# fluidex/plonkit

Measured on AMD Instinct MI355X. Metric: G1 MSM throughput at 2^20 terms per GPU (KZG commitment of the PLONK prover), higher is better.
Workload: dtype u256 (BN254 Fr/Fq Montgomery; 9x29-bit limbs in registers, v_mad_u64_u32); 1 GPU; Pippenger G1 MSM (KZG commitment), 2^20 uniform scalars per GPU, tau=42 monomial SRS sharded by rank (BASELINE configs[1]); terms_per_gpu=1048576, parallelism=srs-shard x1 + all_gather of partial sums, exchange=none (one GPU), pipeline_depth=3, settle_steps=0, comm_ranks=1

## Files before the change

### plonkit_amd/csrc/ec29_dev.h

```cpp
#pragma once
#include "field29_dev.h"
#include "ec_dev.h"

namespace plk {

struct AffW { FqW9 x, y; };
struct alignas(16) XyzzW { FqW9 x, y, zz, zzz; };

#define WM(a, b) mulw<FqW>((a), (b))
#define WS(a) sqrw<FqW>((a))
#define WMA(a, b, c, d) mul2addw<FqW>((a), (b), (c), (d))
#define LM(a, b) mulw_os<FqW>((a), (b))
#define LS(a) sqrw_os<FqW>((a))
#define LMA(a, b, c, d) mul2addw_os<FqW>((a), (b), (c), (d))

PLK_HD bool is_inf(const XyzzW &p) { return w_all_zero(p.zz); }
PLK_HD bool is_inf(const AffW &p) { return w_all_zero(p.x) && w_all_zero(p.y); }
PLK_HD XyzzW xyzzw_identity() { XyzzW r; r.x = w_zero<FqW>(); r.y = w_zero<FqW>(); r.zz = w_zero<FqW>(); r.zzz = w_zero<FqW>(); return r; }

PLK_HD XyzzW xyzzw_double_affine(const FqW9 &x, const FqW9 &y) {
    FqW9 u = addn(y, y), v = WS(u), w = WM(u, v), s = WM(x, v);
    FqW9 xx = WS(x), m = normw(addw(addw(xx, xx), xx));
    XyzzW r;
    r.x = sub4(WS(m), addn(s, s));
    r.y = WMA(m, sub6(s, r.x), y, neg2(w));
    r.zz = v; r.zzz = w;
    return r;
}

PLK_HD XyzzW xyzzw_double(const XyzzW &p) {
    if (is_inf(p)) return p;
    FqW9 u = addn(p.y, p.y), v = LS(u), w = LM(u, v), s = LM(p.x, v);
    FqW9 xx = LS(p.x), m = normw(addw(addw(xx, xx), xx));
    XyzzW r;
    r.x = sub4(LS(m), addn(s, s));
    r.y = LMA(m, sub6(s, r.x), p.y, neg2(w));
    r.zz = LM(v, p.zz); r.zzz = LM(w, p.zzz);
    return r;
}

PLK_HD void xyzzw_add(XyzzW &a, const XyzzW &b);
PLK_HD void xyzzw_add_mixed_special(XyzzW &acc, const AffW &q, bool neg_q, const FqW9 &p, const FqW9 &r) {
    if (is_zero_mod_p(p)) {
        if (is_zero_mod_p(r)) acc = xyzzw_double_affine(q.x, neg_q ? neg2(q.y) : q.y);
        else acc = xyzzw_identity();
        return;
    }
    XyzzW t; t.x = q.x; t.y = neg_q ? neg2(q.y) : q.y; t.zz = w_one<FqW>(); t.zzz = w_one<FqW>();
    xyzzw_add(acc, t);
}

PLK_HD void xyzzw_add_mixed(XyzzW &acc, const AffW &q, bool neg_q) {
    if (is_inf(q)) return;
    if (is_inf(acc)) { acc.x = q.x; acc.y = neg_q ? neg2(q.y) : q.y; acc.zz = w_one<FqW>(); acc.zzz = w_one<FqW>(); return; }
    FqW9 u2, s2;
    mulw2<FqW>(q.x, acc.zz, q.y, acc.zzz, u2, s2);
    FqW9 p = sub6(u2, acc.x);
    FqW9 r;
    {
        const uint32_t m = neg_q ? 0xffffffffu : 0u;
#pragma unroll
        for (int i = 0; i < 9; i++) r.l[i] = FqW::PAD8[i] - acc.y.l[i] + ((s2.l[i] ^ m) - m);
        r = normw(r);
    }
    if (maybe_zero_mod_p(p)) {
        xyzzw_add_mixed_special(acc, q, neg_q, p, r);
        return;
    }
    FqW9 pp, rr, ppp, qq;
    sqrw2<FqW>(p, r, pp, rr);
    mulw2<FqW>(p, pp, acc.x, pp, ppp, qq);
    FqW9 x3;
    {
#pragma unroll
        for (int i = 0; i < 9; i++) x3.l[i] = rr.l[i] + FqW::PAD4[i] - ppp.l[i] - 2 * qq.l[i];
        x3 = normw(x3);
    }
    FqW9 zz3, zzz3;
    mulw2<FqW>(acc.zz, pp, acc.zzz, ppp, zz3, zzz3);
    acc.y = WMA(r, sub6(qq, x3), acc.y, neg2(ppp));
    acc.x = x3;
    acc.zz = zz3;
    acc.zzz = zzz3;
}

PLK_HD void xyzzw_add_mixed_flag(XyzzW &acc, bool &fresh, const AffW &q, bool neg_q) {
    if (fresh) { acc.x = q.x; acc.y = neg_q ? neg2(q.y) : q.y; acc.zz = w_one<FqW>(); acc.zzz = w_one<FqW>(); fresh = false; return; }
    FqW9 p, r, yq;
    {
        FqW9 ax, ay;
#pragma unroll
        for (int i = 0; i < 9; i++) {
            ax.l[i] = FqW::PAD6[i] - acc.x.l[i];
            ay.l[i] = FqW::PAD8[i] - acc.y.l[i];
            yq.l[i] = neg_q ? FqW::PAD2[i] - q.y.l[i] : q.y.l[i];
        }
        mulw2_add<FqW>(q.x, acc.zz, ax, yq, acc.zzz, ay, p, r);
    }
    if (maybe_zero_mod_p(p)) {
        AffW t; t.x = q.x; t.y = normw(yq);
        xyzzw_add_mixed_special(acc, t, false, p, r);
        fresh = is_inf(acc);
        return;
    }
    FqW9 pp, rr, ppp, qq;
    sqrw2<FqW>(p, r, pp, rr);
    mulw2<FqW>(p, pp, acc.x, pp, ppp, qq);
    FqW9 x3;
    {
#pragma unroll
        for (int i = 0; i < 9; i++) x3.l[i] = rr.l[i] + FqW::PAD4[i] - ppp.l[i] - 2 * qq.l[i];
        x3 = normw(x3);
    }
    FqW9 zz3, zzz3;
    mulw2<FqW>(acc.zz, pp, acc.zzz, ppp, zz3, zzz3);
    FqW9 t, nppp;
#pragma unroll
    for (int i = 0; i < 9; i++) { t.l[i] = qq.l[i] + FqW::PAD6N[i] - x3.l[i]; nppp.l[i] = FqW::PAD2N[i] - ppp.l[i]; }
    acc.y = WMA(r, t, acc.y, nppp);
    acc.x = x3;
    acc.zz = zz3;
    acc.zzz = zzz3;
}

PLK_HD void xyzzw_add(XyzzW &a, const XyzzW &b) {
    if (is_inf(b)) return;
    if (is_inf(a)) { a = b; return; }
    FqW9 u1 = LM(a.x, b.zz), u2 = LM(b.x, a.zz), s1 = LM(a.y, b.zzz), s2 = LM(b.y, a.zzz);
    FqW9 p = sub2(u2, u1), r = sub2(s2, s1);
    if (is_zero_mod_p(p)) {
        if (is_zero_mod_p(r)) a = xyzzw_double(a);
        else a = xyzzw_identity();
        return;
    }
    FqW9 pp = LS(p), ppp = LM(p, pp), qq = LM(u1, pp);
    FqW9 x3;
    {
        FqW9 rr = LS(r);
#pragma unroll
        for (int i = 0; i < 9; i++) x3.l[i] = rr.l[i] + FqW::PAD4[i] - ppp.l[i] - 2 * qq.l[i];
        x3 = normw(x3);
    }
    a.y = LMA(r, sub6(qq, x3), s1, neg2(ppp));
    a.x = x3;
    a.zz = LM(LM(a.zz, b.zz), pp);
    a.zzz = LM(LM(a.zzz, b.zzz), ppp);
}

PLK_HD void xyzzw_add_pairs(XyzzW &a, const XyzzW &b) {
    if (is_inf(b)) return;
    if (is_inf(a)) { a = b; return; }
    FqW9 u1, s1, p, r;
    mulw2<FqW>(a.x, b.zz, a.y, b.zzz, u1, s1);
    {
        FqW9 nu, ns;
#pragma unroll
        for (int i = 0; i < 9; i++) { nu.l[i] = FqW::PAD2[i] - u1.l[i]; ns.l[i] = FqW::PAD2[i] - s1.l[i]; }
        mulw2_add<FqW>(b.x, a.zz, nu, b.y, a.zzz, ns, p, r);
    }
    if (is_zero_mod_p(p)) {
        if (is_zero_mod_p(r)) a = xyzzw_double(a);
        else a = xyzzw_identity();
        return;
    }
    FqW9 zz12, zzz12;
    mulw2<FqW>(a.zz, b.zz, a.zzz, b.zzz, zz12, zzz12);
    FqW9 pp, rr, ppp, qq;
#pragma unroll
    for (int i = 0; i < 9; i++) { PLK_CHAIN(p.l[i]); PLK_CHAIN(r.l[i]); }
    sqrw2<FqW>(p, r, pp, rr);
    mulw2<FqW>(p, pp, u1, pp, ppp, qq);
    FqW9 x3;
    {
#pragma unroll
        for (int i = 0; i < 9; i++) x3.l[i] = rr.l[i] + FqW::PAD4[i] - ppp.l[i] - 2 * qq.l[i];
        x3 = normw(x3);
    }
    FqW9 t, nppp;
#pragma unroll
    for (int i = 0; i < 9; i++) { t.l[i] = qq.l[i] + FqW::PAD6N[i] - x3.l[i]; nppp.l[i] = FqW::PAD2N[i] - ppp.l[i]; }
    a.y = WMA(r, t, s1, nppp);
    a.x = x3;
    mulw2<FqW>(zz12, pp, zzz12, ppp, a.zz, a.zzz);
}

__device__ __forceinline__ AffW load_affw(const G1Affine *p) {
    AffW r; r.x = unpack<FqW>(load_fp(&p->x)); r.y = unpack<FqW>(load_fp(&p->y)); return r;
}
__device__ __forceinline__ FqW9 load_w(const uint32_t *p) {
    FqW9 r;
    const u32x4 *q = reinterpret_cast<const u32x4 *>(p);
    u32x4 a = q[0], b = q[1];
    r.l[0] = a.x; r.l[1] = a.y; r.l[2] = a.z; r.l[3] = a.w; r.l[4] = b.x; r.l[5] = b.y; r.l[6] = b.z; r.l[7] = b.w; r.l[8] = p[8];
    return r;
}
__device__ __forceinline__ void store_w(uint32_t *p, const FqW9 &v) {
    u32x4 *q = reinterpret_cast<u32x4 *>(p);
    q[0] = u32x4{v.l[0], v.l[1], v.l[2], v.l[3]};
    q[1] = u32x4{v.l[4], v.l[5], v.l[6], v.l[7]};
    p[8] = v.l[8];
}
__device__ __forceinline__ XyzzW load_xyzzw(const XyzzW *p) {
    const uint32_t *w = reinterpret_cast<const uint32_t *>(p);
    XyzzW r;
    FqW9 *c[4] = {&r.x, &r.y, &r.zz, &r.zzz};
    u32x4 tail = *reinterpret_cast<const u32x4 *>(w + 32);
    const uint32_t t[4] = {tail.x, tail.y, tail.z, tail.w};
#pragma unroll
    for (int k = 0; k < 4; k++) {
        const u32x4 *q = reinterpret_cast<const u32x4 *>(w + 8 * k);
        u32x4 a = q[0], b = q[1];
        c[k]->l[0] = a.x; c[k]->l[1] = a.y; c[k]->l[2] = a.z; c[k]->l[3] = a.w;
        c[k]->l[4] = b.x; c[k]->l[5] = b.y; c[k]->l[6] = b.z; c[k]->l[7] = b.w; c[k]->l[8] = t[k];
    }
    return r;
}
__device__ __forceinline__ void store_xyzzw(XyzzW *p, const XyzzW &v) {
    uint32_t *w = reinterpret_cast<uint32_t *>(p);
    const FqW9 *c[4] = {&v.x, &v.y, &v.zz, &v.zzz};
#pragma unroll
    for (int k = 0; k < 4; k++) {
        u32x4 *q = reinterpret_cast<u32x4 *>(w + 8 * k);
        q[0] = u32x4{c[k]->l[0], c[k]->l[1], c[k]->l[2], c[k]->l[3]};
        q[1] = u32x4{c[k]->l[4], c[k]->l[5], c[k]->l[6], c[k]->l[7]};
    }
    *reinterpret_cast<u32x4 *>(w + 32) = u32x4{v.x.l[8], v.y.l[8], v.zz.l[8], v.zzz.l[8]};
}

__device__ __forceinline__ G1Xyzz xyzzw_export(const XyzzW &p) {
    G1Xyzz r;
    if (is_inf(p)) return xyzz_identity();
    r.x = pack<FqParams>(s_from_w(p.x)); r.y = pack<FqParams>(s_from_w(p.y));
    r.zz = pack<FqParams>(s_from_w(p.zz)); r.zzz = pack<FqParams>(s_from_w(p.zzz));
    return r;
}

}
```

### plonkit_amd/csrc/field29_dev.h

```cpp
#pragma once
#include "field_dev.h"
#include <utility>

namespace plk {

template <int... J, class F> __device__ __forceinline__ void static_for_impl(std::integer_sequence<int, J...>, F &&f) { (f(std::integral_constant<int, J>{}), ...); }
template <int N, class F> __device__ __forceinline__ void static_for(F &&f) { static_for_impl(std::make_integer_sequence<int, N>{}, static_cast<F &&>(f)); }

constexpr uint32_t M29 = (1u << 29) - 1;
constexpr uint32_t MULW_A_LIMB_MAX = 3280000000u;

struct FrW {
    static constexpr uint32_t P29[9] = {0x10000001u, 0x1f0fac9fu, 0x0e5c2450u, 0x07d090f3u, 0x1585d283u, 0x02db40c0u, 0x00a6e141u, 0x0e5c2634u, 0x0030644eu};
    static constexpr uint32_t INV29 = 0x0fffffffu;
    static constexpr uint32_t PINV0 = 0x10000001u;
    static constexpr uint32_t ONE_W[9] = {0x0fffff57u, 0x1ea70ab4u, 0x052c068bu, 0x17504f49u, 0x0aa8075bu, 0x1d4240ceu, 0x11d54c07u, 0x052ac7a8u, 0x000dc836u};
    static constexpr uint32_t W_FROM_S[9] = {0x0fffead7u, 0x1d5444f4u, 0x04438aa5u, 0x03b4d096u, 0x134c84dau, 0x0e92d304u, 0x14cb95b3u, 0x041b9d3du, 0x00058003u};
    static constexpr uint32_t S_FROM_W[9] = {0x0ffffffbu, 0x04b1a0e2u, 0x18334a6bu, 0x18ed2b3eu, 0x1462e36fu, 0x11b7bc3cu, 0x1cbd99bau, 0x183340fbu, 0x000e0a77u};
    static constexpr uint32_t PAD2[9] = {0x80000002u, 0x9e1f593bu, 0x9cb8489du, 0x8fa121e2u, 0x8b0ba502u, 0x85b6817du, 0x814dc27eu, 0x9cb84c64u, 0x0060c898u};
    static constexpr uint32_t PAD4[9] = {0x80000004u, 0x9c3eb27au, 0x9970913fu, 0x9f4243c9u, 0x96174a08u, 0x8b6d02feu, 0x829b8500u, 0x997098ccu, 0x00c19135u};
    static constexpr uint32_t PAD6[9] = {0x80000006u, 0x9a5e0bb9u, 0x9628d9e1u, 0x8ee365b0u, 0x8122ef0fu, 0x91238480u, 0x83e94782u, 0x9628e534u, 0x012259d2u};
    static constexpr uint32_t PAD8[9] = {0x80000008u, 0x987d64f8u, 0x92e12283u, 0x9e848797u, 0x8c2e9415u, 0x96da0601u, 0x85370a04u, 0x92e1319cu, 0x0183226fu};
};

// ... 95 lines not shown
#pragma unroll
    for (int i = 0; i < 9; i++) r.l[i] = WP::PAD2[i] - a.l[i];
    return normw(r);
}
template <class WP> PLK_HD W9<WP> addn(const W9<WP> &a, const W9<WP> &b) { return normw(addw(a, b)); }

#if defined(__HIP_DEVICE_COMPILE__)
#define PLK_CHAIN(acc) asm("" : "+v"(acc))
#else
#define PLK_CHAIN(acc) do { } while (0)
#endif
#define PLK_MONT_LOW(k)  { _Pragma("unroll") for (int i = 0; i < (k); i++) { acc += (uint64_t)m[i] * WP::P29[(k) - i]; PLK_CHAIN(acc); } \
                           m[k] = ((uint32_t)acc * WP::INV29) & M29; acc += (uint64_t)m[k] * WP::P29[0]; acc >>= 29; }
#define PLK_MONT_HIGH(k) { _Pragma("unroll") for (int i = (k) - 8; i <= 8; i++) { acc += (uint64_t)m[i] * WP::P29[(k) - i]; PLK_CHAIN(acc); } \
                           r.l[(k) - 9] = (uint32_t)acc & M29; acc >>= 29; }
template <class WP>
PLK_HD W9<WP> mulw(const W9<WP> &a, const W9<WP> &b) {
    uint32_t m[9];
    W9<WP> r;
    uint64_t acc = 0;
#pragma unroll
    for (int k = 0; k < 9; k++) {
#pragma unroll
        for (int i = 0; i <= k; i++) { acc += (uint64_t)a.l[k - i] * b.l[i]; PLK_CHAIN(acc); }
        PLK_MONT_LOW(k)
    }
#pragma unroll
    for (int k = 9; k < 17; k++) {
#pragma unroll
        for (int i = k - 8; i <= 8; i++) { acc += (uint64_t)a.l[k - i] * b.l[i]; PLK_CHAIN(acc); }
        PLK_MONT_HIGH(k)
    }
    r.l[8] = (uint32_t)acc;
    return r;
}
#define PLK_MONT_LOW2(k)  { _Pragma("unroll") for (int i = 0; i < (k); i++) { acc0 += (uint64_t)m0[i] * WP::P29[(k) - i]; PLK_CHAIN(acc0); acc1 += (uint64_t)m1[i] * WP::P29[(k) - i]; PLK_CHAIN(acc1); } \
                            m0[k] = ((uint32_t)acc0 * WP::INV29) & M29; m1[k] = ((uint32_t)acc1 * WP::INV29) & M29; \
                            acc0 += (uint64_t)m0[k] * WP::P29[0]; acc1 += (uint64_t)m1[k] * WP::P29[0]; acc0 >>= 29; acc1 >>= 29; }
#define PLK_MONT_HIGH2(k) { _Pragma("unroll") for (int i = (k) - 8; i <= 8; i++) { acc0 += (uint64_t)m0[i] * WP::P29[(k) - i]; PLK_CHAIN(acc0); acc1 += (uint64_t)m1[i] * WP::P29[(k) - i]; PLK_CHAIN(acc1); } \
                            r0.l[(k) - 9] = (uint32_t)acc0 & M29; r1.l[(k) - 9] = (uint32_t)acc1 & M29; acc0 >>= 29; acc1 >>= 29; }
template <class WP>
PLK_HD void mulw2(const W9<WP> &a0, const W9<WP> &b0, const W9<WP> &a1, const W9<WP> &b1, W9<WP> &r0, W9<WP> &r1) {
    uint32_t m0[9], m1[9];
    uint64_t acc0 = 0, acc1 = 0;
#pragma unroll
    for (int k = 0; k < 9; k++) {
#pragma unroll
        for (int i = 0; i <= k; i++) { acc0 += (uint64_t)a0.l[k - i] * b0.l[i]; PLK_CHAIN(acc0); acc1 += (uint64_t)a1.l[k - i] * b1.l[i]; PLK_CHAIN(acc1); }
        PLK_MONT_LOW2(k)
    }
#pragma unroll
    for (int k = 9; k < 17; k++) {
#pragma unroll
        for (int i = k - 8; i <= 8; i++) { acc0 += (uint64_t)a0.l[k - i] * b0.l[i]; PLK_CHAIN(acc0); acc1 += (uint64_t)a1.l[k - i] * b1.l[i]; PLK_CHAIN(acc1); }
        PLK_MONT_HIGH2(k)
    }
    r0.l[8] = (uint32_t)acc0; r1.l[8] = (uint32_t)acc1;
}
template <class WP>
PLK_HD void sqrw2(const W9<WP> &x0, const W9<WP> &x1, W9<WP> &r0, W9<WP> &r1) {
    uint32_t m0[9], m1[9], d0[9], d1[9];
    uint64_t acc0 = 0, acc1 = 0;
#pragma unroll
    for (int j = 0; j < 9; j++) { d0[j] = x0.l[j] << 1; d1[j] = x1.l[j] << 1; }
#pragma unroll
    for (int k = 0; k < 9; k++) {
#pragma unroll
        for (int i = 0; 2 * i < k; i++) { acc0 += (uint64_t)d0[k - i] * x0.l[i]; PLK_CHAIN(acc0); acc1 += (uint64_t)d1[k - i] * x1.l[i]; PLK_CHAIN(acc1); }
        if (k % 2 == 0) { acc0 += (uint64_t)x0.l[k / 2] * x0.l[k / 2]; PLK_CHAIN(acc0); acc1 += (uint64_t)x1.l[k / 2] * x1.l[k / 2]; PLK_CHAIN(acc1); }
        PLK_MONT_LOW2(k)
    }
#pragma unroll
    for (int k = 9; k < 17; k++) {
#pragma unroll
        for (int i = k - 8; 2 * i < k; i++) { acc0 += (uint64_t)d0[k - i] * x0.l[i]; PLK_CHAIN(acc0); acc1 += (uint64_t)d1[k - i] * x1.l[i]; PLK_CHAIN(acc1); }
        if (k % 2 == 0) { acc0 += (uint64_t)x0.l[k / 2] * x0.l[k / 2]; PLK_CHAIN(acc0); acc1 += (uint64_t)x1.l[k / 2] * x1.l[k / 2]; PLK_CHAIN(acc1); }
        PLK_MONT_HIGH2(k)
    }
    r0.l[8] = (uint32_t)acc0; r1.l[8] = (uint32_t)acc1;
}
#if defined(__HIP_DEVICE_COMPILE__)
#define PLK_ADDEND(acc, x) { uint32_t one_ = 1; asm("" : "+s"(one_)); (acc) += (uint64_t)(x) * one_; }
#else
#define PLK_ADDEND(acc, x) { (acc) += (uint64_t)(x); }
#endif
#define PLK_MONT_HIGH2_ADD(k) { _Pragma("unroll") for (int i = (k) - 8; i <= 8; i++) { acc0 += (uint64_t)m0[i] * WP::P29[(k) - i]; PLK_CHAIN(acc0); acc1 += (uint64_t)m1[i] * WP::P29[(k) - i]; PLK_CHAIN(acc1); } \
                                PLK_ADDEND(acc0, A0.l[(k) - 9]); PLK_ADDEND(acc1, A1.l[(k) - 9]); \
                                r0.l[(k) - 9] = (uint32_t)acc0 & M29; r1.l[(k) - 9] = (uint32_t)acc1 & M29; acc0 >>= 29; acc1 >>= 29; }
template <class WP>
PLK_HD void mulw2_add(const W9<WP> &a0, const W9<WP> &b0, const W9<WP> &A0, const W9<WP> &a1, const W9<WP> &b1, const W9<WP> &A1, W9<WP> &r0, W9<WP> &r1) {
    uint32_t m0[9], m1[9];
    uint64_t acc0 = 0, acc1 = 0;
#pragma unroll
    for (int k = 0; k < 9; k++) {
#pragma unroll
        for (int i = 0; i <= k; i++) { acc0 += (uint64_t)a0.l[k - i] * b0.l[i]; PLK_CHAIN(acc0); acc1 += (uint64_t)a1.l[k - i] * b1.l[i]; PLK_CHAIN(acc1); }
        PLK_MONT_LOW2(k)
    }
#pragma unroll
    for (int k = 9; k < 17; k++) {
#pragma unroll
        for (int i = k - 8; i <= 8; i++) { acc0 += (uint64_t)a0.l[k - i] * b0.l[i]; PLK_CHAIN(acc0); acc1 += (uint64_t)a1.l[k - i] * b1.l[i]; PLK_CHAIN(acc1); }
        PLK_MONT_HIGH2_ADD(k)
    }
    r0.l[8] = (uint32_t)acc0 + A0.l[8]; r1.l[8] = (uint32_t)acc1 + A1.l[8];
}

template <class WP>
PLK_HD W9<WP> sqrw(const W9<WP> &a) {
    uint32_t m[9], a2[9];
    W9<WP> r;
    uint64_t acc = 0;
#pragma unroll
    for (int j = 0; j < 9; j++) a2[j] = a.l[j] << 1;
#pragma unroll
    for (int k = 0; k < 9; k++) {
#pragma unroll
        for (int i = 0; 2 * i < k; i++) { acc += (uint64_t)a2[k - i] * a.l[i]; PLK_CHAIN(acc); }
        if (k % 2 == 0) { acc += (uint64_t)a.l[k / 2] * a.l[k / 2]; PLK_CHAIN(acc); }
        PLK_MONT_LOW(k)
    }
#pragma unroll
    for (int k = 9; k < 17; k++) {
#pragma unroll
        for (int i = k - 8; 2 * i < k; i++) { acc += (uint64_t)a2[k - i] * a.l[i]; PLK_CHAIN(acc); }
        if (k % 2 == 0) { acc += (uint64_t)a.l[k / 2] * a.l[k / 2]; PLK_CHAIN(acc); }
        PLK_MONT_HIGH(k)
    }
    r.l[8] = (uint32_t)acc;
    return r;
}

template <class WP>
PLK_HD W9<WP> mul2addw(const W9<WP> &a, const W9<WP> &b, const W9<WP> &c, const W9<WP> &d) {
    uint32_t m[9];
    W9<WP> r;
    uint64_t acc = 0;
#pragma unroll
    for (int k = 0; k < 9; k++) {
#pragma unroll
        for (int i = 0; i <= k; i++) { acc += (uint64_t)a.l[k - i] * b.l[i]; PLK_CHAIN(acc); acc += (uint64_t)c.l[k - i] * d.l[i]; PLK_CHAIN(acc); }
        PLK_MONT_LOW(k)
    }
#pragma unroll
    for (int k = 9; k < 17; k++) {
#pragma unroll
        for (int i = k - 8; i <= 8; i++) { acc += (uint64_t)a.l[k - i] * b.l[i]; PLK_CHAIN(acc); acc += (uint64_t)c.l[k - i] * d.l[i]; PLK_CHAIN(acc); }
        PLK_MONT_HIGH(k)
    }
    r.l[8] = (uint32_t)acc;
    return r;
}

constexpr uint32_t MULTW3_X_LIMB_MAX = 3600000000u;
template <class WP> struct Tw3 { uint32_t w[3][9]; };
template <class WP>
PLK_HD W9<WP> mul_tw3(const W9<WP> &x, const Tw3<WP> &t) {
    uint32_t m[3];
    W9<WP> r;
    uint64_t acc = 0;
#pragma unroll
    for (int k = 0; k < 11; k++) {
#pragma unroll
        for (int i = 0; i < 3; i++) {
            if (k - i < 0 || k - i > 8) continue;
#pragma unroll
            for (int q = 0; q < 3; q++) { acc += (uint64_t)x.l[3 * q + i] * t.w[q][k - i]; PLK_CHAIN(acc); }
        }
#pragma unroll
        for (int i = 0; i < 3; i++) {
            if (i >= k || k - i > 8) continue;
            acc += (uint64_t)m[i] * WP::P29[k - i]; PLK_CHAIN(acc);
        }
        if (k < 3) { m[k] = ((uint32_t)acc * WP::INV29) & M29; acc += (uint64_t)m[k] * WP::P29[0]; }
        else r.l[k - 3] = (uint32_t)acc & M29;
        acc >>= 29;
    }
    r.l[8] = (uint32_t)acc;
    return r;
}
template <class WP>
PLK_HD void mul_tw3_2(const W9<WP> &x0, const W9<WP> &x1, const Tw3<WP> &t, W9<WP> &r0, W9<WP> &r1) {
    uint32_t m0[3], m1[3];
    uint64_t acc0 = 0, acc1 = 0;
#pragma unroll
    for (int k = 0; k < 11; k++) {
#pragma unroll
        for (int i = 0; i < 3; i++) {
            if (k - i < 0 || k - i > 8) continue;
#pragma unroll
            for (int q = 0; q < 3; q++) {
                acc0 += (uint64_t)x0.l[3 * q + i] * t.w[q][k - i]; PLK_CHAIN(acc0);
                acc1 += (uint64_t)x1.l[3 * q + i] * t.w[q][k - i]; PLK_CHAIN(acc1);
            }
        }
#pragma unroll
        for (int i = 0; i < 3; i++) {
            if (i >= k || k - i > 8) continue;
            acc0 += (uint64_t)m0[i] * WP::P29[k - i]; PLK_CHAIN(acc0);
            acc1 += (uint64_t)m1[i] * WP::P29[k - i]; PLK_CHAIN(acc1);
        }
        if (k < 3) {
            m0[k] = ((uint32_t)acc0 * WP::INV29) & M29; m1[k] = ((uint32_t)acc1 * WP::INV29) & M29;
            acc0 += (uint64_t)m0[k] * WP::P29[0]; acc1 += (uint64_t)m1[k] * WP::P29[0];
        } else { r0.l[k - 3] = (uint32_t)acc0 & M29; r1.l[k - 3] = (uint32_t)acc1 & M29; }
        acc0 >>= 29; acc1 >>= 29;
    }
    r0.l[8] = (uint32_t)acc0; r1.l[8] = (uint32_t)acc1;
}
template <class WP>
PLK_HD Tw3<WP> make_tw3(const W9<WP> &w_dom_w) {
    W9<WP> e87 = w_zero<WP>(), e174 = w_zero<WP>();
    e87.l[3] = 1; e174.l[6] = 1;
    const W9<WP> w0 = csub_p(mulw(w_dom_w, e87)), w1 = csub_p(mulw(w_dom_w, e174));
    Tw3<WP> t;
    for (int i = 0; i < 9; i++) { t.w[0][i] = w0.l[i]; t.w[1][i] = w1.l[i]; t.w[2][i] = w_dom_w.l[i]; }
    return t;
}

template <class WP>
PLK_HD W9<WP> mulw_os(const W9<WP> &a, const W9<WP> &b) {
    uint64_t t[10];
#pragma unroll
    for (int j = 0; j < 10; j++) t[j] = 0;
#pragma unroll
    for (int i = 0; i < 9; i++) {
#pragma unroll
        for (int j = 0; j < 9; j++) t[j] += (uint64_t)a.l[j] * b.l[i];
        const uint32_t m = ((uint32_t)t[0] * WP::INV29) & M29;
#pragma unroll
        for (int j = 0; j < 9; j++) t[j] += (uint64_t)m * WP::P29[j];
        const uint64_t c = t[0] >> 29;
#pragma unroll
        for (int j = 0; j < 9; j++) t[j] = t[j + 1];
        t[0] += c;
        t[9] = 0;
    }
    W9<WP> r;
    uint64_t c = 0;
#pragma unroll
    for (int j = 0; j < 8; j++) { uint64_t s = t[j] + c; r.l[j] = (uint32_t)s & M29; c = s >> 29; }
    r.l[8] = (uint32_t)(t[8] + c);
    return r;
}
template <class WP>
PLK_HD W9<WP> sqrw_os(const W9<WP> &a) {
    uint64_t t[10];
    uint32_t a2[9];
#pragma unroll
    for (int j = 0; j < 10; j++) t[j] = 0;
#pragma unroll
    for (int j = 0; j < 9; j++) a2[j] = a.l[j] << 1;
#pragma unroll
    for (int i = 0; i < 9; i++) {
        t[i] += (uint64_t)a.l[i] * a.l[i];
#pragma unroll
        for (int j = i + 1; j < 9; j++) t[j] += (uint64_t)a2[j] * a.l[i];
        const uint32_t m = ((uint32_t)t[0] * WP::INV29) & M29;
#pragma unroll
        for (int j = 0; j < 9; j++) t[j] += (uint64_t)m * WP::P29[j];
        const uint64_t c = t[0] >> 29;
#pragma unroll
        for (int j = 0; j < 9; j++) t[j] = t[j + 1];
        t[0] += c;
        t[9] = 0;
    }
    W9<WP> r;
    uint64_t c = 0;
#pragma unroll
    for (int j = 0; j < 8; j++) { uint64_t s = t[j] + c; r.l[j] = (uint32_t)s & M29; c = s >> 29; }
    r.l[8] = (uint32_t)(t[8] + c);
    return r;
}

template <class WP>
PLK_HD W9<WP> mul2addw_os(const W9<WP> &a, const W9<WP> &b, const W9<WP> &c, const W9<WP> &d) {
    uint64_t t[10];
#pragma unroll
    for (int j = 0; j < 10; j++) t[j] = 0;
#pragma unroll
    for (int i = 0; i < 9; i++) {
#pragma unroll
        for (int j = 0; j < 9; j++) t[j] += (uint64_t)a.l[j] * b.l[i];
#pragma unroll
        for (int j = 0; j < 9; j++) t[j] += (uint64_t)c.l[j] * d.l[i];
        const uint32_t m = ((uint32_t)t[0] * WP::INV29) & M29;
#pragma unroll
        for (int j = 0; j < 9; j++) t[j] += (uint64_t)m * WP::P29[j];
        const uint64_t cy = t[0] >> 29;
#pragma unroll
        for (int j = 0; j < 9; j++) t[j] = t[j + 1];
        t[0] += cy;
        t[9] = 0;
    }
    W9<WP> r;
    uint64_t cy = 0;
#pragma unroll
    for (int j = 0; j < 8; j++) { uint64_t s = t[j] + cy; r.l[j] = (uint32_t)s & M29; cy = s >> 29; }
    r.l[8] = (uint32_t)(t[8] + cy);
    return r;
}

template <class WP>
PLK_HD W9<WP> csub_p(const W9<WP> &a) {
    int32_t d[9];
    int32_t c = 0;
// ... 91 lines not shown
```

### plonkit_amd/csrc/msm_accumulate.hip

```cpp
#include "msm_shape.h"
#include "ec29_quad_dev.h"
#include <atomic>

namespace plk {

template <uint32_t FB, int MINW = 2, bool OWNED = false, bool Q_MAY_BE_INF = true>
__global__ void __launch_bounds__(MSM_THREADS, MINW) msm_accumulate(const G1Affine *bases, const uint32_t *entries,
                                                                  const uint32_t *bin_start, const uint32_t *task_start,
                                                                  XyzzW *partials, uint32_t *task_meta, MsmParams p) {
    constexpr uint32_t FINE = Shape<FB>::FINE, SLOT_PRIMARY = Shape<FB>::SLOT_PRIMARY, SLOT_HEAD = Shape<FB>::SLOT_HEAD,
                       SLOT_TAIL = Shape<FB>::SLOT_TAIL, SLOTS_PER_TASK = Shape<FB>::SLOTS_PER_TASK, META_PER_TASK = Shape<FB>::META_PER_TASK;
    extern __shared__ uint32_t sorted[];
    __shared__ uint32_t cnt[FINE], start[FINE + 1], cursor[FINE], max_cnt;
    const uint32_t tid = threadIdx.x, task = blockIdx.x;
    const uint32_t total_bins = p.batch * p.groups * p.nbins;
    if (task >= task_start[total_bins]) return;
    uint32_t blo = 0, bhi = total_bins;
    if (task < total_bins && task_start[task] <= task && task_start[task + 1] > task) { blo = task; bhi = task + 1; }
    while (bhi - blo > 1) { uint32_t mid = (blo + bhi) >> 1; if (task_start[mid] <= task) blo = mid; else bhi = mid; }
    const uint32_t bin = blo, slice = task - task_start[bin];
    const uint32_t bs = bin_start[bin], be = bin_start[bin + 1];
    const uint32_t k_bin = task_start[bin + 1] - task_start[bin], per = (be - bs + k_bin - 1) / k_bin;
    const uint32_t s = bs + slice * per < be ? bs + slice * per : be, e = (s + per < be) ? s + per : be, nc = e - s;

    if (tid < FINE) { cnt[tid] = 0; cursor[tid] = 0; }
    __syncthreads();
    constexpr uint32_t PER_LANE = CHUNK / MSM_THREADS;
    uint32_t ent[PER_LANE];
#pragma unroll
    for (uint32_t k = 0; k < PER_LANE; k++) { const uint32_t idx = tid + k * MSM_THREADS; ent[k] = idx < nc ? entries[s + idx] : 0u; }
    const uint32_t wave_first = (tid & ~63u);
    uint32_t f0, diff = 0;
    {
        const uint32_t e0 = __builtin_amdgcn_readfirstlane(ent[0]);
        f0 = e0 & (FINE - 1);
#pragma unroll
        for (uint32_t k = 0; k < PER_LANE; k++) if (tid + k * MSM_THREADS < nc) diff |= (ent[k] ^ e0) & (FINE - 1);
    }
    const bool wave_hot = wave_first < nc && __ballot(diff != 0) == 0;
    uint32_t wave_n = 0;
    if (wave_hot) {
#pragma unroll
        for (uint32_t k = 0; k < PER_LANE; k++) {
            const uint32_t b0 = wave_first + k * MSM_THREADS;
            wave_n += b0 >= nc ? 0u : (nc - b0 < 64u ? nc - b0 : 64u);
        }
        if ((tid & 63) == 0) atomicAdd(&cnt[f0], wave_n);
    } else {
#pragma unroll
        for (uint32_t k = 0; k < PER_LANE; k++) if (tid + k * MSM_THREADS < nc) atomicAdd(&cnt[ent[k] & (FINE - 1)], 1u);
    }
    __syncthreads();
    if (tid < 64) {
        constexpr uint32_t PER = FINE / 64;
        uint32_t own[PER], sum = 0;
#pragma unroll
        for (uint32_t k = 0; k < PER; k++) { own[k] = cnt[PER * tid + k]; sum += own[k]; }
        uint32_t v = sum;
        for (int off = 1; off < 64; off <<= 1) { uint32_t t = __shfl_up(v, off); if ((int)tid >= off) v += t; }
        uint32_t run = v - sum;
#pragma unroll
        for (uint32_t k = 0; k < PER; k++) { start[PER * tid + k] = run; run += own[k]; }
        if (tid == 63) start[FINE] = v;
        if (OWNED) {
            uint32_t mx = own[0];
#pragma unroll
            for (uint32_t k = 1; k < PER; k++) mx = own[k] > mx ? own[k] : mx;
            for (int off = 1; off < 64; off <<= 1) { const uint32_t t = __shfl_xor(mx, off); mx = t > mx ? t : mx; }
            if (tid == 0) max_cnt = mx;
        }
    }
    __syncthreads();
    uint32_t *meta = task_meta + (size_t)task * META_PER_TASK;
    const uint32_t mu = (nc + MSM_THREADS - 1) / MSM_THREADS;
    const bool owned = OWNED && FINE * 4 == MSM_THREADS && max_cnt <= 8 * mu + 24;
    if (tid <= FINE) meta[tid] = start[tid];
    if (tid == 0) meta[FINE + 1] = nc | (owned ? TASK_OWNED_BIT : 0u);
    if (wave_hot) {
        uint32_t base = 0;
        if ((tid & 63) == 0) base = atomicAdd(&cursor[f0], wave_n);
        base = start[f0] + __builtin_amdgcn_readfirstlane(base);
#pragma unroll
        for (uint32_t k = 0; k < PER_LANE; k++)
            if (tid + k * MSM_THREADS < nc) sorted[base + k * 64 + (tid & 63)] = ent[k];
    } else {
#pragma unroll
        for (uint32_t k = 0; k < PER_LANE; k++)
            if (tid + k * MSM_THREADS < nc) { const uint32_t f = ent[k] & (FINE - 1); sorted[start[f] + atomicAdd(&cursor[f], 1u)] = ent[k]; }
    }
    __syncthreads();
    if (nc == 0) return;
    XyzzW *out = partials + (size_t)task * SLOTS_PER_TASK;
    const uint32_t imask = (1u << p.nbits) - 1;
    auto point_of = [&](uint32_t entry) -> const G1Affine * {
        const uint32_t t = entry >> 8;
        return bases + (size_t)(t >> p.nbits) * p.copy_stride + (t & imask);
    };
    if constexpr (!OWNED && !Q_MAY_BE_INF) {
        const uint32_t lo = tid * mu < nc ? tid * mu : nc, hi = lo + mu < nc ? lo + mu : nc;
        if (lo >= hi) return;
        uint32_t en = sorted[lo];
        G1Affine pt = load_affine(point_of(en));
        uint32_t bend = start[(en & (FINE - 1)) + 1];
        XyzzW acc = xyzzw_identity();
        bool fresh = true, first_run = true;
        for (uint32_t i = lo; i < hi; i++) {
            const uint32_t e_cur = en;
            AffW cur; cur.x = unpack<FqW>(pt.x); cur.y = unpack<FqW>(pt.y);
            if (i + 1 < hi) { en = sorted[i + 1]; pt = load_affine(point_of(en)); }
            if (i == bend) {
                const uint32_t b = sorted[i - 1] & (FINE - 1);
                const bool from_prev = first_run && (start[b] < tid * mu);
                store_xyzzw(out + (from_prev ? SLOT_HEAD + tid : SLOT_PRIMARY + b), acc);
                acc = xyzzw_identity(); fresh = true; first_run = false;
                bend = start[(e_cur & (FINE - 1)) + 1];
            }
            xyzzw_add_mixed_flag(acc, fresh, cur, (e_cur & 0x80u) != 0);
        }
        const uint32_t b = sorted[hi - 1] & (FINE - 1);
        const bool from_prev = first_run && (start[b] < tid * mu), into_next = bend > hi;
        store_xyzzw(out + (from_prev ? SLOT_HEAD + tid : (into_next ? SLOT_TAIL + tid : SLOT_PRIMARY + b)), acc);
        return;
    }
    const bool own = OWNED && owned;
    const uint32_t step = own ? 4u : 1u;
    uint32_t lo, hi;
    if (own) { lo = start[tid >> 2] + (tid & 3u); hi = start[(tid >> 2) + 1]; }
    else {
        lo = tid * mu < nc ? tid * mu : nc; hi = lo + mu < nc ? lo + mu : nc;
        if (lo >= hi) return;
    }
    uint32_t en = 0, b = tid >> 2, bend = 0xffffffffu, run_start = lo;
    G1Affine pt;
    if (lo < hi) { en = sorted[lo]; pt = load_affine(point_of(en)); }
    if (!own) { b = en & (FINE - 1); bend = start[b + 1]; }
    XyzzW acc = xyzzw_identity();
    for (uint32_t i = lo; i < hi; i += step) {
        const uint32_t e_cur = en;
        AffW cur; cur.x = unpack<FqW>(pt.x); cur.y = unpack<FqW>(pt.y);
        if (i + step < hi) { en = sorted[i + step]; pt = load_affine(point_of(en)); }
        if (i == bend) {
            const bool from_prev = (run_start == lo) && (start[b] < lo);
            store_xyzzw(out + (from_prev ? SLOT_HEAD + tid : SLOT_PRIMARY + b), acc);
            acc = xyzzw_identity();
            run_start = i; b = e_cur & (FINE - 1); bend = start[b + 1];
        }
        xyzzw_add_mixed(acc, cur, (e_cur & 0x80u) != 0);
    }
    if (OWNED && own) {
        const uint32_t role = tid & 3u;
        const FqW9 c1 = quad_distribute<1>(acc, role), c2 = quad_distribute<2>(acc, role), c3 = quad_distribute<3>(acc, role);
        FqW9 X = quad_distribute<0>(acc, role);
        for (int k = 1; k < 4; k++) X = xyzzw_add_dist(X, wsel(k == 1, c1, wsel(k == 2, c2, c3)), role);
        if (start[b + 1] > start[b]) store_coord(out + SLOT_PRIMARY + b, role, X);
        return;
    }
    const bool from_prev = (run_start == lo) && (start[b] < lo), into_next = bend > hi;
    store_xyzzw(out + (from_prev ? SLOT_HEAD + tid : (into_next ? SLOT_TAIL + tid : SLOT_PRIMARY + b)), acc);
}


int32_t msm_accumulate_prepare() {
    static std::atomic<bool> attr_set{false};
    if (attr_set) return PLK_OK;
    PLK_HIP(hipFuncSetAttribute(reinterpret_cast<const void *>(msm_accumulate<FINE_BITS>), hipFuncAttributeMaxDynamicSharedMemorySize, CHUNK * sizeof(uint32_t)));
    PLK_HIP(hipFuncSetAttribute(reinterpret_cast<const void *>(msm_accumulate<FINE_BITS, 2, true>), hipFuncAttributeMaxDynamicSharedMemorySize, CHUNK * sizeof(uint32_t)));
    PLK_HIP(hipFuncSetAttribute(reinterpret_cast<const void *>(msm_accumulate<FINE_BITS, 2, false, false>), hipFuncAttributeMaxDynamicSharedMemorySize, CHUNK * sizeof(uint32_t)));
    attr_set = true;
    return PLK_OK;
}

void msm_accumulate_launch(int variant, bool no_inf, uint32_t max_tasks, hipStream_t stream, const G1Affine *bases, const uint32_t *entries,
                           const uint32_t *bin_start, const uint32_t *task_start, XyzzW *partials, uint32_t *task_meta, const MsmParams &p) {
    const size_t lds = CHUNK * sizeof(uint32_t);
    if (variant == 2)
        hipLaunchKernelGGL((msm_accumulate<FINE_BITS, 2, true>), dim3(max_tasks), dim3(MSM_THREADS), lds, stream, bases, entries, bin_start, task_start, partials, task_meta, p);
    else if (no_inf)
        hipLaunchKernelGGL((msm_accumulate<FINE_BITS, 2, false, false>), dim3(max_tasks), dim3(MSM_THREADS), lds, stream, bases, entries, bin_start, task_start, partials, task_meta, p);
    else
        hipLaunchKernelGGL((msm_accumulate<FINE_BITS>), dim3(max_tasks), dim3(MSM_THREADS), lds, stream, bases, entries, bin_start, task_start, partials, task_meta, p);
}

}
```

Measured before the change: 918.3 Mscalar·mul/s.

## Use lazy Montgomery digits and negated-XY accumulator in bucket mixed adds

Adds lazy-reduction variants of the 29-bit-limb Montgomery multiply kernels. They skip masking the quotient digit, and compile-time limb-bound checks prove that the 64-bit columns cannot overflow. The hot bucket-accumulation path now keeps its accumulator with X and Y negated, so the padded subtractions before the mixed-add multiply are dropped. The result is flipped back at each store. The pairwise add also uses the lazy kernels, and the next point's unpack is moved ahead in the loop. This trades extra template complexity and flip costs at bucket boundaries for fewer ALU ops per point add.

```diff
diff --git a/plonkit_amd/csrc/ec29_dev.h b/plonkit_amd/csrc/ec29_dev.h
--- a/plonkit_amd/csrc/ec29_dev.h
+++ b/plonkit_amd/csrc/ec29_dev.h
@@ -10,9 +10,14 @@
 #define WM(a, b) mulw<FqW>((a), (b))
 #define WS(a) sqrw<FqW>((a))
 #define WMA(a, b, c, d) mul2addw<FqW>((a), (b), (c), (d))
+#define WMA_LZ(a, b, c, d) mul2addw_lz<FqW, LZ_ALL, LbNorm, LbT, LbNorm, LbNppp>((a), (b), (c), (d))
 #define LM(a, b) mulw_os<FqW>((a), (b))
 #define LS(a) sqrw_os<FqW>((a))
 #define LMA(a, b, c, d) mul2addw_os<FqW>((a), (b), (c), (d))
+
+struct LbSignedY { static constexpr Limbs9 B = lb_max(LbNorm::B, lb_of(FqW::PAD2)); };
+struct LbT { static constexpr Limbs9 B = lb_plus(lb_of(FqW::PAD6N), M29); };
+struct LbNppp { static constexpr Limbs9 B = lb_of(FqW::PAD2N); };
 
 PLK_HD bool is_inf(const XyzzW &p) { return w_all_zero(p.zz); }
 PLK_HD bool is_inf(const AffW &p) { return w_all_zero(p.x) && w_all_zero(p.y); }
@@ -84,44 +89,56 @@
     acc.zzz = zzz3;
 }
 
-PLK_HD void xyzzw_add_mixed_flag(XyzzW &acc, bool &fresh, const AffW &q, bool neg_q) {
-    if (fresh) { acc.x = q.x; acc.y = neg_q ? neg2(q.y) : q.y; acc.zz = w_one<FqW>(); acc.zzz = w_one<FqW>(); fresh = false; return; }
+PLK_HD XyzzW xyzzw_flip_xy(const XyzzW &a) { XyzzW r = a; r.x = sub6(w_zero<FqW>(), a.x); r.y = sub6(w_zero<FqW>(), a.y); return r; }
+template <bool NXY>
+PLK_HD void xyzzw_add_mixed_flag_impl(XyzzW &acc, bool &fresh, const AffW &q, bool neg_q) {
+    if (fresh) {
+        if constexpr (NXY) { acc.x = neg2(q.x); acc.y = neg_q ? q.y : neg2(q.y); }
+        else { acc.x = q.x; acc.y = neg_q ? neg2(q.y) : q.y; }
+        acc.zz = w_one<FqW>(); acc.zzz = w_one<FqW>(); fresh = false; return;
+    }
     FqW9 p, r, yq;
-    {
+#pragma unroll
+    for (int i = 0; i < 9; i++) yq.l[i] = neg_q ? FqW::PAD2[i] - q.y.l[i] : q.y.l[i];
+    if constexpr (NXY) mulw2_add_lz<FqW, LZ_ALL, LZ_ALL, LbNorm, LbNorm, LbNorm, LbSignedY, LbNorm, LbNorm>(q.x, acc.zz, acc.x, yq, acc.zzz, acc.y, p, r);
+    else {
         FqW9 ax, ay;
 #pragma unroll
         for (int i = 0; i < 9; i++) {
             ax.l[i] = FqW::PAD6[i] - acc.x.l[i];
             ay.l[i] = FqW::PAD8[i] - acc.y.l[i];
-            yq.l[i] = neg_q ? FqW::PAD2[i] - q.y.l[i] : q.y.l[i];
         }
-        mulw2_add<FqW>(q.x, acc.zz, ax, yq, acc.zzz, ay, p, r);
+        mulw2_add_lz<FqW, LZ_ALL, LZ_ALL, LbNorm, LbNorm, LbAny, LbSignedY, LbNorm, LbAny>(q.x, acc.zz, ax, yq, acc.zzz, ay, p, r);
     }
     if (maybe_zero_mod_p(p)) {
         AffW t; t.x = q.x; t.y = normw(yq);
+        if constexpr (NXY) acc = xyzzw_flip_xy(acc);
         xyzzw_add_mixed_special(acc, t, false, p, r);
         fresh = is_inf(acc);
+        if constexpr (NXY) acc = xyzzw_flip_xy(acc);
         return;
     }
     FqW9 pp, rr, ppp, qq;
-    sqrw2<FqW>(p, r, pp, rr);
-    mulw2<FqW>(p, pp, acc.x, pp, ppp, qq);
-    FqW9 x3;
-    {
-#pragma unroll
-        for (int i = 0; i < 9; i++) x3.l[i] = rr.l[i] + FqW::PAD4[i] - ppp.l[i] - 2 * qq.l[i];
+    sqrw2_lz<FqW, LZ_ALL, LZ_ALL, LbNorm, LbNorm>(p, r, pp, rr);
+    mulw2_lz<FqW, LZ_ALL, LZ_ALL, LbNorm, LbNorm, LbNorm, LbNorm>(p, pp, acc.x, pp, ppp, qq);
+    FqW9 x3;
+    {
+#pragma unroll
+        for (int i = 0; i < 9; i++) x3.l[i] = NXY ? ppp.l[i] + FqW::PAD4[i] - rr.l[i] - 2 * qq.l[i] : rr.l[i] + FqW::PAD4[i] - ppp.l[i] - 2 * qq.l[i];
         x3 = normw(x3);
     }
     FqW9 zz3, zzz3;
-    mulw2<FqW>(acc.zz, pp, acc.zzz, ppp, zz3, zzz3);
+    mulw2_lz<FqW, LZ_ALL, LZ_ALL, LbNorm, LbNorm, LbNorm, LbNorm>(acc.zz, pp, acc.zzz, ppp, zz3, zzz3);
     FqW9 t, nppp;
 #pragma unroll
     for (int i = 0; i < 9; i++) { t.l[i] = qq.l[i] + FqW::PAD6N[i] - x3.l[i]; nppp.l[i] = FqW::PAD2N[i] - ppp.l[i]; }
-    acc.y = WMA(r, t, acc.y, nppp);
+    acc.y = WMA_LZ(r, t, acc.y, nppp);
     acc.x = x3;
     acc.zz = zz3;
     acc.zzz = zzz3;
 }
+PLK_HD void xyzzw_add_mixed_flag(XyzzW &acc, bool &fresh, const AffW &q, bool neg_q) { xyzzw_add_mixed_flag_impl<false>(acc, fresh, q, neg_q); }
+PLK_HD void xyzzw_add_mixed_nflag(XyzzW &acc, bool &fresh, const AffW &q, bool neg_q) { xyzzw_add_mixed_flag_impl<true>(acc, fresh, q, neg_q); }
 
 PLK_HD void xyzzw_add(XyzzW &a, const XyzzW &b) {
     if (is_inf(b)) return;
@@ -151,12 +168,12 @@
     if (is_inf(b)) return;
     if (is_inf(a)) { a = b; return; }
     FqW9 u1, s1, p, r;
-    mulw2<FqW>(a.x, b.zz, a.y, b.zzz, u1, s1);
+    mulw2_lz<FqW, LZ_ALL, LZ_ALL, LbNorm, LbNorm, LbNorm, LbNorm>(a.x, b.zz, a.y, b.zzz, u1, s1);
     {
         FqW9 nu, ns;
 #pragma unroll
         for (int i = 0; i < 9; i++) { nu.l[i] = FqW::PAD2[i] - u1.l[i]; ns.l[i] = FqW::PAD2[i] - s1.l[i]; }
-        mulw2_add<FqW>(b.x, a.zz, nu, b.y, a.zzz, ns, p, r);
+        mulw2_add_lz<FqW, LZ_ALL, LZ_ALL, LbNorm, LbNorm, LbAny, LbNorm, LbNorm, LbAny>(b.x, a.zz, nu, b.y, a.zzz, ns, p, r);
     }
     if (is_zero_mod_p(p)) {
         if (is_zero_mod_p(r)) a = xyzzw_double(a);
@@ -164,12 +181,12 @@
         return;
     }
     FqW9 zz12, zzz12;
-    mulw2<FqW>(a.zz, b.zz, a.zzz, b.zzz, zz12, zzz12);
+    mulw2_lz<FqW, LZ_ALL, LZ_ALL, LbNorm, LbNorm, LbNorm, LbNorm>(a.zz, b.zz, a.zzz, b.zzz, zz12, zzz12);
     FqW9 pp, rr, ppp, qq;
 #pragma unroll
     for (int i = 0; i < 9; i++) { PLK_CHAIN(p.l[i]); PLK_CHAIN(r.l[i]); }
-    sqrw2<FqW>(p, r, pp, rr);
-    mulw2<FqW>(p, pp, u1, pp, ppp, qq);
+    sqrw2_lz<FqW, LZ_ALL, LZ_ALL, LbNorm, LbNorm>(p, r, pp, rr);
+    mulw2_lz<FqW, LZ_ALL, LZ_ALL, LbNorm, LbNorm, LbNorm, LbNorm>(p, pp, u1, pp, ppp, qq);
     FqW9 x3;
     {
 #pragma unroll
@@ -179,9 +196,9 @@
     FqW9 t, nppp;
 #pragma unroll
     for (int i = 0; i < 9; i++) { t.l[i] = qq.l[i] + FqW::PAD6N[i] - x3.l[i]; nppp.l[i] = FqW::PAD2N[i] - ppp.l[i]; }
-    a.y = WMA(r, t, s1, nppp);
+    a.y = WMA_LZ(r, t, s1, nppp);
     a.x = x3;
-    mulw2<FqW>(zz12, pp, zzz12, ppp, a.zz, a.zzz);
+    mulw2_lz<FqW, LZ_ALL, LZ_ALL, LbNorm, LbNorm, LbNorm, LbNorm>(zz12, pp, zzz12, ppp, a.zz, a.zzz);
 }
 
 __device__ __forceinline__ AffW load_affw(const G1Affine *p) {
diff --git a/plonkit_amd/csrc/field29_dev.h b/plonkit_amd/csrc/field29_dev.h
--- a/plonkit_amd/csrc/field29_dev.h
+++ b/plonkit_amd/csrc/field29_dev.h
@@ -271,6 +271,127 @@
     return r;
 }
 
+struct Limbs9 { uint32_t l[9]; };
+constexpr Limbs9 lb_uniform(uint32_t v) { return Limbs9{{v, v, v, v, v, v, v, v, v}}; }
+constexpr Limbs9 lb_of(const uint32_t (&a)[9]) { return Limbs9{{a[0], a[1], a[2], a[3], a[4], a[5], a[6], a[7], a[8]}}; }
+constexpr Limbs9 lb_plus(const Limbs9 &a, uint32_t v) { Limbs9 r{}; for (int i = 0; i < 9; i++) r.l[i] = a.l[i] + v; return r; }
+constexpr bool lb_below(const Limbs9 &a, uint32_t v) { for (int i = 0; i < 9; i++) if (a.l[i] >= v) return false; return true; }
+constexpr Limbs9 lb_max(const Limbs9 &a, const Limbs9 &b) { Limbs9 r{}; for (int i = 0; i < 9; i++) r.l[i] = a.l[i] > b.l[i] ? a.l[i] : b.l[i]; return r; }
+struct LbNone { static constexpr Limbs9 B = lb_uniform(0); };
+struct LbNorm { static constexpr Limbs9 B = lb_uniform(M29); };
+struct LbAny { static constexpr Limbs9 B = lb_uniform(0xffffffffu); };
+constexpr unsigned LZ_ALL = 0xffu;
+constexpr bool lazy_digit(unsigned lz, int k) { return k < 8 && ((lz >> k) & 1u); }
+struct ColBound { uint64_t worst; bool fits; };
+constexpr ColBound lazy_col_bound(const Limbs9 &a, const Limbs9 &b, const Limbs9 &c, const Limbs9 &d, const Limbs9 &addend, const uint32_t (&p)[9], unsigned lz) {
+    uint64_t carry = 0, worst = 0;
+    bool fits = true;
+    for (int k = 0; k < 17; k++) {
+        uint64_t s = carry;
+        for (int i = (k < 9 ? 0 : k - 8); i <= (k < 9 ? k : 8); i++) {
+            fits &= !__builtin_add_overflow(s, (uint64_t)a.l[k - i] * b.l[i], &s);
+            fits &= !__builtin_add_overflow(s, (uint64_t)c.l[k - i] * d.l[i], &s);
+            fits &= !__builtin_add_overflow(s, (uint64_t)(lazy_digit(lz, i) ? 0xffffffffu : M29) * p[k - i], &s);
+        }
+        if (k >= 9) fits &= !__builtin_add_overflow(s, (uint64_t)addend.l[k - 9], &s);
+        if (s > worst) worst = s;
+        carry = s >> 29;
+    }
+    return ColBound{worst, fits};
+}
+#define PLK_LZ_DIGIT(LZ, k, acc) (lazy_digit((LZ), (k)) ? (uint32_t)(acc) * WP::INV29 : ((uint32_t)(acc) * WP::INV29) & M29)
+#define PLK_MONT_LOW_LZ(k)   { _Pragma("unroll") for (int i = 0; i < (k); i++) { acc += (uint64_t)m[i] * WP::P29[(k) - i]; PLK_CHAIN(acc); } \
+                               m[k] = PLK_LZ_DIGIT(LZ, k, acc); acc += (uint64_t)m[k] * WP::P29[0]; acc >>= 29; }
+#define PLK_MONT_LOW2_LZ(k)  { _Pragma("unroll") for (int i = 0; i < (k); i++) { acc0 += (uint64_t)m0[i] * WP::P29[(k) - i]; PLK_CHAIN(acc0); acc1 += (uint64_t)m1[i] * WP::P29[(k) - i]; PLK_CHAIN(acc1); } \
+                               m0[k] = PLK_LZ_DIGIT(LZ0, k, acc0); m1[k] = PLK_LZ_DIGIT(LZ1, k, acc1); \
+                               acc0 += (uint64_t)m0[k] * WP::P29[0]; acc1 += (uint64_t)m1[k] * WP::P29[0]; acc0 >>= 29; acc1 >>= 29; }
+template <class WP, unsigned LZ0, unsigned LZ1, class LA0, class LB0, class LA1, class LB1>
+PLK_HD void mulw2_lz(const W9<WP> &a0, const W9<WP> &b0, const W9<WP> &a1, const W9<WP> &b1, W9<WP> &r0, W9<WP> &r1) {
+    static_assert(lazy_col_bound(LA0::B, LB0::B, LbNone::B, LbNone::B, LbNone::B, WP::P29, LZ0).fits, "mulw2_lz: a column of chain 0 can exceed 64 bits");
+    static_assert(lazy_col_bound(LA1::B, LB1::B, LbNone::B, LbNone::B, LbNone::B, WP::P29, LZ1).fits, "mulw2_lz: a column of chain 1 can exceed 64 bits");
+    uint32_t m0[9], m1[9];
+    uint64_t acc0 = 0, acc1 = 0;
+#pragma unroll
+    for (int k = 0; k < 9; k++) {
+#pragma unroll
+        for (int i = 0; i <= k; i++) { acc0 += (uint64_t)a0.l[k - i] * b0.l[i]; PLK_CHAIN(acc0); acc1 += (uint64_t)a1.l[k - i] * b1.l[i]; PLK_CHAIN(acc1); }
+        PLK_MONT_LOW2_LZ(k)
+    }
+#pragma unroll
+    for (int k = 9; k < 17; k++) {
+#pragma unroll
+        for (int i = k - 8; i <= 8; i++) { acc0 += (uint64_t)a0.l[k - i] * b0.l[i]; PLK_CHAIN(acc0); acc1 += (uint64_t)a1.l[k - i] * b1.l[i]; PLK_CHAIN(acc1); }
+        PLK_MONT_HIGH2(k)
+    }
+    r0.l[8] = (uint32_t)acc0; r1.l[8] = (uint32_t)acc1;
+}
+template <class WP, unsigned LZ0, unsigned LZ1, class LX0, class LX1>
+PLK_HD void sqrw2_lz(const W9<WP> &x0, const W9<WP> &x1, W9<WP> &r0, W9<WP> &r1) {
+    static_assert(lazy_col_bound(LX0::B, LX0::B, LbNone::B, LbNone::B, LbNone::B, WP::P29, LZ0).fits, "sqrw2_lz: a column of chain 0 can exceed 64 bits");
+    static_assert(lazy_col_bound(LX1::B, LX1::B, LbNone::B, LbNone::B, LbNone::B, WP::P29, LZ1).fits, "sqrw2_lz: a column of chain 1 can exceed 64 bits");
+    static_assert(lb_below(LX0::B, 1u << 31) && lb_below(LX1::B, 1u << 31), "sqrw2_lz: a doubled limb can exceed 32 bits");
+    uint32_t m0[9], m1[9], d0[9], d1[9];
+    uint64_t acc0 = 0, acc1 = 0;
+#pragma unroll
+    for (int j = 0; j < 9; j++) { d0[j] = x0.l[j] << 1; d1[j] = x1.l[j] << 1; }
+#pragma unroll
+    for (int k = 0; k < 9; k++) {
+#pragma unroll
+        for (int i = 0; 2 * i < k; i++) { acc0 += (uint64_t)d0[k - i] * x0.l[i]; PLK_CHAIN(acc0); acc1 += (uint64_t)d1[k - i] * x1.l[i]; PLK_CHAIN(acc1); }
+        if (k % 2 == 0) { acc0 += (uint64_t)x0.l[k / 2] * x0.l[k / 2]; PLK_CHAIN(acc0); acc1 += (uint64_t)x1.l[k / 2] * x1.l[k / 2]; PLK_CHAIN(acc1); }
+        PLK_MONT_LOW2_LZ(k)
+    }
+#pragma unroll
+    for (int k = 9; k < 17; k++) {
+#pragma unroll
+        for (int i = k - 8; 2 * i < k; i++) { acc0 += (uint64_t)d0[k - i] * x0.l[i]; PLK_CHAIN(acc0); acc1 += (uint64_t)d1[k - i] * x1.l[i]; PLK_CHAIN(acc1); }
+        if (k % 2 == 0) { acc0 += (uint64_t)x0.l[k / 2] * x0.l[k / 2]; PLK_CHAIN(acc0); acc1 += (uint64_t)x1.l[k / 2] * x1.l[k / 2]; PLK_CHAIN(acc1); }
+        PLK_MONT_HIGH2(k)
+    }
+    r0.l[8] = (uint32_t)acc0; r1.l[8] = (uint32_t)acc1;
+}
+template <class WP, unsigned LZ0, unsigned LZ1, class LA0, class LB0, class LAD0, class LA1, class LB1, class LAD1>
+PLK_HD void mulw2_add_lz(const W9<WP> &a0, const W9<WP> &b0, const W9<WP> &A0, const W9<WP> &a1, const W9<WP> &b1, const W9<WP> &A1, W9<WP> &r0, W9<WP> &r1) {
+    static_assert(lazy_col_bound(LA0::B, LB0::B, LbNone::B, LbNone::B, LAD0::B, WP::P29, LZ0).fits, "mulw2_add_lz: a column of chain 0 can exceed 64 bits");
+    static_assert(lazy_col_bound(LA1::B, LB1::B, LbNone::B, LbNone::B, LAD1::B, WP::P29, LZ1).fits, "mulw2_add_lz: a column of chain 1 can exceed 64 bits");
+    uint32_t m0[9], m1[9];
+    uint64_t acc0 = 0, acc1 = 0;
+#pragma unroll
+    for (int k = 0; k < 9; k++) {
+#pragma unroll
+        for (int i = 0; i <= k; i++) { acc0 += (uint64_t)a0.l[k - i] * b0.l[i]; PLK_CHAIN(acc0); acc1 += (uint64_t)a1.l[k - i] * b1.l[i]; PLK_CHAIN(acc1); }
+        PLK_MONT_LOW2_LZ(k)
+    }
+#pragma unroll
+    for (int k = 9; k < 17; k++) {
+#pragma unroll
+        for (int i = k - 8; i <= 8; i++) { acc0 += (uint64_t)a0.l[k - i] * b0.l[i]; PLK_CHAIN(acc0); acc1 += (uint64_t)a1.l[k - i] * b1.l[i]; PLK_CHAIN(acc1); }
+        PLK_MONT_HIGH2_ADD(k)
+    }
+    r0.l[8] = (uint32_t)acc0 + A0.l[8]; r1.l[8] = (uint32_t)acc1 + A1.l[8];
+}
+template <class WP, unsigned LZ, class LA, class LB, class LC, class LD>
+PLK_HD W9<WP> mul2addw_lz(const W9<WP> &a, const W9<WP> &b, const W9<WP> &c, const W9<WP> &d) {
+    static_assert(lazy_col_bound(LA::B, LB::B, LC::B, LD::B, LbNone::B, WP::P29, LZ).fits, "mul2addw_lz: a column can exceed 64 bits");
+    uint32_t m[9];
+    W9<WP> r;
+    uint64_t acc = 0;
+#pragma unroll
+    for (int k = 0; k < 9; k++) {
+#pragma unroll
+        for (int i = 0; i <= k; i++) { acc += (uint64_t)a.l[k - i] * b.l[i]; PLK_CHAIN(acc); acc += (uint64_t)c.l[k - i] * d.l[i]; PLK_CHAIN(acc); }
+        PLK_MONT_LOW_LZ(k)
+    }
+#pragma unroll
+    for (int k = 9; k < 17; k++) {
+#pragma unroll
+        for (int i = k - 8; i <= 8; i++) { acc += (uint64_t)a.l[k - i] * b.l[i]; PLK_CHAIN(acc); acc += (uint64_t)c.l[k - i] * d.l[i]; PLK_CHAIN(acc); }
+        PLK_MONT_HIGH(k)
+    }
+    r.l[8] = (uint32_t)acc;
+    return r;
+}
+
 constexpr uint32_t MULTW3_X_LIMB_MAX = 3600000000u;
 template <class WP> struct Tw3 { uint32_t w[3][9]; };
 template <class WP>
diff --git a/plonkit_amd/csrc/msm_accumulate.hip b/plonkit_amd/csrc/msm_accumulate.hip
--- a/plonkit_amd/csrc/msm_accumulate.hip
+++ b/plonkit_amd/csrc/msm_accumulate.hip
@@ -103,23 +103,25 @@
         G1Affine pt = load_affine(point_of(en));
         uint32_t bend = start[(en & (FINE - 1)) + 1];
         XyzzW acc = xyzzw_identity();
+        AffW nxt; nxt.x = unpack<FqW>(pt.x); nxt.y = unpack<FqW>(pt.y);
         bool fresh = true, first_run = true;
         for (uint32_t i = lo; i < hi; i++) {
             const uint32_t e_cur = en;
-            AffW cur; cur.x = unpack<FqW>(pt.x); cur.y = unpack<FqW>(pt.y);
+            const AffW cur = nxt;
             if (i + 1 < hi) { en = sorted[i + 1]; pt = load_affine(point_of(en)); }
             if (i == bend) {
                 const uint32_t b = sorted[i - 1] & (FINE - 1);
                 const bool from_prev = first_run && (start[b] < tid * mu);
-                store_xyzzw(out + (from_prev ? SLOT_HEAD + tid : SLOT_PRIMARY + b), acc);
+                store_xyzzw(out + (from_prev ? SLOT_HEAD + tid : SLOT_PRIMARY + b), xyzzw_flip_xy(acc));
                 acc = xyzzw_identity(); fresh = true; first_run = false;
                 bend = start[(e_cur & (FINE - 1)) + 1];
             }
-            xyzzw_add_mixed_flag(acc, fresh, cur, (e_cur & 0x80u) != 0);
+            xyzzw_add_mixed_nflag(acc, fresh, cur, (e_cur & 0x80u) != 0);
+            nxt.x = unpack<FqW>(pt.x); nxt.y = unpack<FqW>(pt.y);
         }
         const uint32_t b = sorted[hi - 1] & (FINE - 1);
         const bool from_prev = first_run && (start[b] < tid * mu), into_next = bend > hi;
-        store_xyzzw(out + (from_prev ? SLOT_HEAD + tid : (into_next ? SLOT_TAIL + tid : SLOT_PRIMARY + b)), acc);
+        store_xyzzw(out + (from_prev ? SLOT_HEAD + tid : (into_next ? SLOT_TAIL + tid : SLOT_PRIMARY + b)), xyzzw_flip_xy(acc));
         return;
     }
     const bool own = OWNED && owned;
```

New measurement: 954.4 Mscalar·mul/s, median of 6. 1.04x the previous value.
